# wuxiaolang/Cube_SLAM_wu

Measured on AMD Instinct MI355X. Metric: frames/sec detect_cuboid, higher is better.
Workload: dtype f64

## Files before the change

### cube_slam_wu_amd/csrc/cs_geom.h

```cpp
#pragma once
#include "cs_atan2.h"

namespace cs {

struct V2 {
  double x, y;
};

CS_HD V2 v2(double x, double y) { return V2{x, y}; }
CS_HD double v2_dist(V2 a, V2 b) {
  double dx = a.x - b.x, dy = a.y - b.y;
  return __builtin_sqrt(dx * dx + dy * dy);
}
CS_HD double v2_dist2(V2 a, V2 b) {
  double dx = a.x - b.x, dy = a.y - b.y;
  return dx * dx + dy * dy;
}
static inline double cs_next_up(double x) { long long b = cs_bits(x); return cs_from_bits(b + 1); }
static inline double cs_next_down(double x) { long long b = cs_bits(x); return cs_from_bits(b - 1); }
static inline double sqrt_lt_bound(double t) {
  if (!(t > 0)) return 0.0;
  if (t == __builtin_huge_val()) return t;
  double c = t * t;
  if (c == __builtin_huge_val()) c = 1.7976931348623157e308;
  while (c > 0 && __builtin_sqrt(c) >= t) c = cs_next_down(c);
  while (__builtin_sqrt(c) < t) { if (c >= 1.7976931348623157e308) return __builtin_huge_val(); c = cs_next_up(c); }
  return c;
}
static inline double sqrt_le_bound(double t) {
  if (t != t) return __builtin_huge_val();
  if (t < 0) return -1.0;
  if (t == __builtin_huge_val()) return t;
  const double lt = sqrt_lt_bound(cs_next_up(t));
  if (lt == __builtin_huge_val()) return 1.7976931348623157e308;
  return lt > 0 ? cs_next_down(lt) : 0.0;
}
CS_HD double dmin(double a, double b) { return (b < a) ? b : a; }
CS_HD double dmax(double a, double b) { return (a < b) ? b : a; }
CS_HD double dabs(double a) { return __builtin_fabs(a); }

#define CS_PI 3.14159265358979323846

CS_HD double normalize_to_pi(double a) {
  if (a > CS_PI / 2) return a - CS_PI;
  else if (a < -CS_PI / 2) return a + CS_PI;
  return a;
}

CS_HD bool inside_box(V2 p, double l, double t, double r, double b) { return l <= p.x && p.x <= r && t <= p.y && p.y <= b; }

CS_HD V2 ray_hit_vertical(V2 s, V2 e, double bx, double by0, double by1) {
  V2 hit = v2(-1, -1);
  double dx = e.x - s.x, dy = e.y - s.y;
  if (by0 == by1) {
    double lambd = (by0 - s.y) / dy;
    if (lambd >= 0) {
      V2 t = v2(s.x + lambd * dx, s.y + lambd * dy);
      if ((bx <= t.x) && (t.x <= bx)) { hit = t; hit.y = by0; }
    }
  }
  double lambd = (bx - s.x) / dx;
  if (lambd >= 0) {
    V2 t = v2(s.x + lambd * dx, s.y + lambd * dy);
    if ((by0 <= t.y) && (t.y <= by1)) { hit = t; hit.x = bx; }
  }
  return hit;
}

CS_HD V2 ray_hit_horizontal(V2 s, V2 e, double by, double bx0, double bx1) {
  V2 hit = v2(-1, -1);
  double dx = e.x - s.x, dy = e.y - s.y;
  double lambd = (by - s.y) / dy;
  if (lambd >= 0) {
    V2 t = v2(s.x + lambd * dx, s.y + lambd * dy);
    if ((bx0 <= t.x) && (t.x <= bx1)) { hit = t; hit.y = by; }
  }
  if (bx0 == bx1) {
    double l2 = (bx0 - s.x) / dx;
    if (l2 >= 0) {
      V2 t = v2(s.x + l2 * dx, s.y + l2 * dy);
      if ((by <= t.y) && (t.y <= by)) { hit = t; hit.x = bx0; }
    }
  }
  return hit;
}

CS_HD V2 line_intersect(V2 a1, V2 a2, V2 b1, V2 b2) {
  double X2_X1 = a2.x - a1.x, Y2_Y1 = a2.y - a1.y;
  double X4_X3 = b2.x - b1.x, Y4_Y3 = b2.y - b1.y;
  double X1_X3 = a1.x - b1.x, Y1_Y3 = a1.y - b1.y;
  double u_a = (X4_X3 * Y1_Y3 - Y4_Y3 * X1_X3) / (Y4_Y3 * X2_X1 - X4_X3 * Y2_Y1);
  return v2((a1.x + X2_X1 * u_a) * 1.0, (a1.y + Y2_Y1 * u_a) * 1.0);
}

struct BoxGeom {
  int left, top, right, down;
  int el, et, er, eb;
};

CS_HD int build_corners(const BoxGeom& g, V2 vp1, V2 vp2, V2 vp3, double top_x, int config_id, double short_sq_bound, V2 c[8]) {
  V2 c1 = v2(top_x, (double)g.top);
  int vp1_pos = 0;
  V2 c2 = ray_hit_vertical(vp1, c1, (double)g.right, (double)g.top, (double)g.down);
  if (c2.x == -1) {
    c2 = ray_hit_vertical(vp1, c1, (double)g.left, (double)g.top, (double)g.down);
    if (c2.x != -1) vp1_pos = 2;
  } else {
    vp1_pos = 1;
  }
  if (!(vp1_pos > 0)) return 0;
  if (v2_dist2(c1, c2) < short_sq_bound) return 0;
  V2 c3, c4;
  if (config_id == 1) {
    if (vp1_pos == 1) c4 = ray_hit_vertical(vp2, c1, (double)g.left, (double)g.top, (double)g.down);
    else c4 = ray_hit_vertical(vp2, c1, (double)g.right, (double)g.top, (double)g.down);
    if (c4.y == -1) return 0;
    if (v2_dist2(c1, c4) < short_sq_bound) return 0;
    c3 = line_intersect(vp2, c2, vp1, c4);
    if (!inside_box(c3, g.left, g.top, g.right, g.down)) return 0;
    if ((v2_dist2(c3, c4) < short_sq_bound) || (v2_dist2(c3, c2) < short_sq_bound)) return 0;
  } else {
    if (vp1_pos == 1) c3 = ray_hit_vertical(vp2, c2, (double)g.left, (double)g.top, (double)g.down);
    else c3 = ray_hit_vertical(vp2, c2, (double)g.right, (double)g.top, (double)g.down);
    if (c3.y == -1) return 0;
    if (v2_dist2(c2, c3) < short_sq_bound) return 0;
    c4 = line_intersect(vp1, c3, vp2, c1);
    if (!inside_box(c4, g.left, g.et, g.right, g.eb)) return 0;
    if ((v2_dist2(c3, c4) < short_sq_bound) || (v2_dist2(c4, c1) < short_sq_bound)) return 0;
  }
  V2 c5 = ray_hit_horizontal(vp3, c3, (double)g.down, (double)g.left, (double)g.right);
  if (c5.y == -1) return 0;
  if (v2_dist2(c3, c5) < short_sq_bound) return 0;
  V2 c6 = line_intersect(vp2, c5, vp3, c2);
  if (!inside_box(c6, g.el, g.et, g.er, g.eb)) return 0;
  if ((v2_dist2(c6, c2) < short_sq_bound) || (v2_dist2(c6, c5) < short_sq_bound)) return 0;
  V2 c7 = line_intersect(vp1, c6, vp3, c1);
  if (!inside_box(c7, g.el, g.et, g.er, g.eb)) return 0;
  if ((v2_dist2(c7, c1) < short_sq_bound) || (v2_dist2(c7, c6) < short_sq_bound)) return 0;
  V2 c8 = line_intersect(vp1, c5, vp2, c7);
  if (!inside_box(c8, g.el, g.et, g.er, g.eb)) return 0;
  if ((v2_dist2(c8, c4) < short_sq_bound) || (v2_dist2(c8, c5) < short_sq_bound) || (v2_dist2(c8, c7) < short_sq_bound)) return 0;
  c[0] = c1; c[1] = c2; c[2] = c3; c[3] = c4; c[4] = c5; c[5] = c6; c[6] = c7; c[7] = c8;
  return vp1_pos;
}

CS_HD void rebuild_accepted_corners(const BoxGeom& g, V2 vp1, V2 vp2, V2 vp3, double top_x, int config_id, int vp1_pos, V2 c[8]) {
  const V2 c1 = v2(top_x, (double)g.top);
  const bool right_first = vp1_pos == 1;
  const double side1 = (double)(right_first ? g.right : g.left), side2 = (double)(right_first ? g.left : g.right);
  const bool k1 = config_id == 1;
  V2 c2;
  { const double dx = c1.x - vp1.x, dy = c1.y - vp1.y, lambd = (side1 - vp1.x) / dx; c2 = v2(side1, vp1.y + lambd * dy); }
  const V2 P = k1 ? c1 : c2;
  V2 H;
  { const double dx = P.x - vp2.x, dy = P.y - vp2.y, lambd = (side2 - vp2.x) / dx; H = v2(side2, vp2.y + lambd * dy); }
  const V2 L = line_intersect(k1 ? vp2 : vp1, k1 ? c2 : H, k1 ? vp1 : vp2, k1 ? H : c1);
  const V2 c3 = k1 ? L : H, c4 = k1 ? H : L;
  V2 c5;
  { const double dx = c3.x - vp3.x, dy = c3.y - vp3.y, lambd = ((double)g.down - vp3.y) / dy; c5 = v2(vp3.x + lambd * dx, (double)g.down); }
  const V2 c6 = line_intersect(vp2, c5, vp3, c2);
  const V2 c7 = line_intersect(vp1, c6, vp3, c1);
  const V2 c8 = line_intersect(vp1, c5, vp2, c7);
  c[0] = c1; c[1] = c2; c[2] = c3; c[3] = c4; c[4] = c5; c[5] = c6; c[6] = c7; c[7] = c8;
}

struct RpPose {
  double KinvR[9];
  double R[9];
  double t[3];
  double plane[4];
  double roll, pitch;
};

CS_HD void plane_hit_world(const double* R, const double* t, const double* invK, const double plane[4], double px, double py, double out[3]) {
  double ray[3];
  for (int i = 0; i < 3; i++) ray[i] = (invK[3 * i + 0] * px + invK[3 * i + 1] * py) + invK[3 * i + 2] * 1.0;
  double den = (plane[0] * ray[0] + plane[1] * ray[1]) + plane[2] * ray[2];
  double frac = -plane[3] / den;
  double p[3] = {frac * ray[0], frac * ray[1], frac * ray[2]};
  double w = ((0.0 * p[0] + 0.0 * p[1]) + 0.0 * p[2]) + 1.0 * 1.0;
  for (int i = 0; i < 3; i++) {
    double v = ((R[3 * i + 0] * p[0] + R[3 * i + 1] * p[1]) + R[3 * i + 2] * p[2]) + t[i] * 1.0;
    out[i] = (w != w) ? w : v;
  }
}

CS_HD void lift_to_3d(const V2 c[8], const double* R, const double* t, const double* invK, const double ground_plane[4], double pos[3], double scale[3]) {
  double g[4][3];
  for (int k = 0; k < 4; k++) plane_hit_world(R, t, invK, ground_plane, c[4 + k].x, c[4 + k].y, g[k]);
  double d03[3] = {g[0][0] - g[3][0], g[0][1] - g[3][1], g[0][2] - g[3][2]};
  double d01[3] = {g[0][0] - g[1][0], g[0][1] - g[1][1], g[0][2] - g[1][2]};
  double length_half = __builtin_sqrt((d03[0] * d03[0] + d03[1] * d03[1]) + d03[2] * d03[2]) / 2;
  double width_half = __builtin_sqrt((d01[0] * d01[0] + d01[1] * d01[1]) + d01[2] * d01[2]) / 2;
  double n[3] = {d01[1] * 1.0 - d01[2] * 0.0, d01[2] * 0.0 - d01[0] * 1.0, d01[0] * 0.0 - d01[1] * 0.0};
  double nn = __builtin_sqrt((n[0] * n[0] + n[1] * n[1]) + n[2] * n[2]);
  for (int i = 0; i < 3; i++) n[i] /= nn;
  double dist = -((n[0] * g[0][0] + n[1] * g[0][1]) + n[2] * g[0][2]);
  double pw[4] = {n[0], n[1], n[2], dist};
  if (dist < 0) for (int i = 0; i < 4; i++) pw[i] = -pw[i];
  double ps[4];
  for (int i = 0; i < 3; i++) ps[i] = ((R[0 + i] * pw[0] + R[3 + i] * pw[1]) + R[6 + i] * pw[2]) + 0.0 * pw[3];
  ps[3] = ((t[0] * pw[0] + t[1] * pw[1]) + t[2] * pw[2]) + 1.0 * pw[3];
  double top[3];
  plane_hit_world(R, t, invK, ps, c[1].x, c[1].y, top);
  double height_half = top[2] / 2;
  pos[0] = (((g[0][0] + g[1][0]) + g[2][0]) + g[3][0]) / 4.0;
  pos[1] = (((g[0][1] + g[1][1]) + g[2][1]) + g[3][1]) / 4.0;
  pos[2] = height_half;
  scale[0] = length_half; scale[1] = width_half; scale[2] = height_half;
}

}
```

### cube_slam_wu_amd/csrc/detect_kernels.hip

```cpp
#include <hip/hip_runtime.h>
#include "cs_hip_util.h"

#include <cstdio>
#include <cstdlib>
#include <cstring>

#include "../../include/cubeslam_hip.h"
#include "detect_types.h"

namespace cs {

__device__ __forceinline__ int wave_uniform_i32(int x) { return __builtin_amdgcn_readfirstlane(x); }
__device__ __forceinline__ long long wave_uniform_i64(long long x) {
  const unsigned lo = (unsigned)__builtin_amdgcn_readfirstlane((int)(unsigned)(x & 0xffffffffll)), hi = (unsigned)__builtin_amdgcn_readfirstlane((int)(x >> 32));
  return (long long)(((unsigned long long)hi << 32) | lo);
}
template <typename T>
__device__ __forceinline__ int find_job_wave(const T* __restrict__ prefix, int n, T elem) {
  const T first = sizeof(T) == 8 ? (T)wave_uniform_i64((long long)elem) : (T)wave_uniform_i32((int)elem);
  int lo = 0, hi = n;
  while (hi - lo > 1) {
    const int mid = (lo + hi) >> 1;
    if (prefix[mid] <= first) lo = mid; else hi = mid;
  }
// ... 123 lines not shown
        ch->dir[lane] = make_float2(cosf((float)a), sinf((float)a));
      }
      __builtin_amdgcn_fence(__ATOMIC_ACQ_REL, "wavefront");
      __builtin_amdgcn_wave_barrier();
      unsigned long long mask[K];
#pragma unroll
      for (int k = 0; k < K; k++) mask[k] = 0;
#pragma unroll 4
      for (int u = 0; u < n; u++) {
        const double2 P = ch->xy[u];
        const float2 ud = ch->dir[u];
#pragma unroll
        for (int k = 0; k < K; k++) {
          const float fx = (float)(P.x - vpx[k]), fy = (float)(P.y - vpy[k]);
          const float cr = fabsf(__builtin_fmaf(fx, ud.y, -(fy * ud.x))), dt = fabsf(__builtin_fmaf(fx, ud.x, fy * ud.y));
          const bool out_for_sure = cr > __builtin_fmaf(tan_f[k], dt, 2.0e-6f * (fabsf(fx) + fabsf(fy)));
          mask[k] |= (unsigned long long)(out_for_sure ? 0 : 1) << u;
        }
      }
#pragma unroll
      for (int k = 0; k < K; k++) {
        unsigned long long mk = lane_on ? mask[k] : 0ull;
        while (__any(mk != 0)) {
          if (mk != 0) {
            const int u = __ffsll((long long)mk) - 1;
            mk &= mk - 1;
            const double2 P = ch->xy[u];
            vp_step(mx, my, c0 + u, P.x, P.y, ch->ang[u], vpx[k], vpy[k], thre[k], thre_f[k], R[k]);
          }
        }
      }
    }
  } else {
    const int mm = lane_on ? m : 0;
    for (int i = 0; i < mm; i++) {
      const double X = mx[i], Y = my[i], A = la[i];
#pragma unroll
      for (int k = 0; k < K; k++) vp_step(mx, my, i, X, Y, A, vpx[k], vpy[k], thre[k], thre_f[k], R[k]);
    }
  }
  const double NaN = __builtin_nan("");
#pragma unroll
  for (int k = 0; k < K; k++) {
    const double ang_hi = R[k].have ? la[R[k].i_hi] : NaN, ang_lo = R[k].have ? la[R[k].i_lo] : NaN;
    out[2 * k] = swapped[k] ? ang_lo : ang_hi;
    out[2 * k + 1] = swapped[k] ? ang_hi : ang_lo;
  }
}

enum { VP3_RPCAP = 32 };

template <int MODE, bool UNIFORM>
__device__ __forceinline__ void vp_support_body(const DetectDeviceView& v, const SweepParams& sp, const JobDesc& jd, int j, long long e, bool on, VpChunk* ch) {
  int rp = 0, y = 0;
  if (on) {
    int local = (int)e - jd.vp_off;
    on = local < jd.RP * jd.Y;
    rp = local / jd.Y; y = local - rp * jd.Y;
  }
  double vpx[3] = {0, 0, 0}, vpy[3] = {0, 0, 0};
  if (on) {
    const RpPose* pose = v.rp + jd.rp_off + rp;
    double cy = v.yaw_cos[jd.yaw_off + y], sy = v.yaw_sin[jd.yaw_off + y];
    const double* A = pose->KinvR;
    double d[3][3] = {{cy, sy, 0.0}, {-sy, cy, 0.0}, {0.0, 0.0, 1.0}};
#pragma unroll
    for (int k = 0; k < 3; k++) {
      double h0 = (A[0] * d[k][0] + A[1] * d[k][1]) + A[2] * d[k][2];
      double h1 = (A[3] * d[k][0] + A[4] * d[k][1]) + A[5] * d[k][2];
      double h2 = (A[6] * d[k][0] + A[7] * d[k][1]) + A[8] * d[k][2];
      vpx[k] = h0 / h2;
      vpy[k] = h1 / h2;
    }
    if (MODE == 0) {
      double* vout = v.vp + 6 * e;
      vout[0] = vpx[0]; vout[1] = vpy[0]; vout[2] = vpx[1]; vout[3] = vpy[1]; vout[4] = vpx[2]; vout[5] = vpy[2];
    }
  }
  const double* mx = v.mid_x + jd.line_off;
  const double* my = v.mid_y + jd.line_off;
  const double* la = v.line_angle + jd.line_off;
  double b6[6];
  const double thre[3] = {sp.vp12_thre_rad, sp.vp12_thre_rad, sp.vp3_thre_rad};
  const bool swapped[3] = {false, true, true};
  vp_support_multi<(MODE == 0 ? 3 : 2), UNIFORM>(mx, my, la, jd.m, ch, vpx, vpy, thre, swapped, on, b6);
  if (!on) return;
  if (MODE == 1) { const double* t3 = v.bound3 + 2 * ((size_t)j * VP3_RPCAP + rp); b6[4] = t3[0]; b6[5] = t3[1]; }
  double* bout = v.bound + 6 * e;
#pragma unroll
  for (int q = 0; q < 6; q++) bout[q] = b6[q];
}

template <int MODE>
__global__ __launch_bounds__(256) void vp_support_kernel(DetectDeviceView v, SweepParams sp, int vp_total) {
  long long e = xcd_virtual_block() * blockDim.x + threadIdx.x;
  const bool on = e < vp_total;
  const int j = find_job_wave<int>(v.vp_prefix, v.n_jobs, on ? (int)e : vp_total - 1);
  const int ju = wave_uniform_i32(j);
  __shared__ VpChunk chunk[4];
  if (__all(j == ju)) vp_support_body<MODE, true>(v, sp, v.jobs[ju], ju, e, on, &chunk[threadIdx.x >> 6]);
  else vp_support_body<MODE, false>(v, sp, v.jobs[j], j, e, on, nullptr);
}

__global__ __launch_bounds__(64) void vp3_support_kernel(DetectDeviceView v, SweepParams sp, int rp_stride) {
  const long long e = (long long)blockIdx.x * 64 + threadIdx.x;
  const int j = (int)(e / rp_stride), rp = (int)(e % rp_stride);
  bool on = j < v.n_jobs;
  JobDesc jd{};
  if (on) { jd = v.jobs[j]; on = rp < jd.RP && jd.Y > 0; }
  double vx = 0, vy = 0;
  if (on) {
    const double* A = (v.rp + jd.rp_off + rp)->KinvR;
    double h0 = (A[0] * 0.0 + A[1] * 0.0) + A[2] * 1.0;
    double h1 = (A[3] * 0.0 + A[4] * 0.0) + A[5] * 1.0;
    double h2 = (A[6] * 0.0 + A[7] * 0.0) + A[8] * 1.0;
    vx = h0 / h2; vy = h1 / h2;
  }
  double o2[2];
  const bool swapped3 = true;
  vp_support_multi<1, false>(v.mid_x + jd.line_off, v.mid_y + jd.line_off, v.line_angle + jd.line_off, on ? jd.m : 0, nullptr, &vx, &vy, &sp.vp3_thre_rad, &swapped3, on, o2);
  if (on) { double* t3 = v.bound3 + 2 * ((size_t)j * VP3_RPCAP + rp); t3[0] = o2[0]; t3[1] = o2[1]; }
}

__global__ __launch_bounds__(256) void vp_points_kernel(DetectDeviceView v, int vp_total) {
  long long e = (long long)blockIdx.x * blockDim.x + threadIdx.x;
  int j = find_job_wave<int>(v.vp_prefix, v.n_jobs, e < vp_total ? (int)e : vp_total - 1);
  if (e >= vp_total) return;
  const JobDesc jd = v.jobs[j];
  int local = (int)e - jd.vp_off;
  if (local >= jd.RP * jd.Y) return;
  int rp = local / jd.Y, y = local - rp * jd.Y;
  const RpPose* pose = v.rp + jd.rp_off + rp;
  double cy = v.yaw_cos[jd.yaw_off + y], sy = v.yaw_sin[jd.yaw_off + y];
  const double* A = pose->KinvR;
  double d[3][3] = {{cy, sy, 0.0}, {-sy, cy, 0.0}, {0.0, 0.0, 1.0}};
  double* vout = v.vp + 6 * e;
#pragma unroll
  for (int k = 0; k < 3; k++) {
    double h0 = (A[0] * d[k][0] + A[1] * d[k][1]) + A[2] * d[k][2];
    double h1 = (A[3] * d[k][0] + A[4] * d[k][1]) + A[5] * d[k][2];
    double h2 = (A[6] * d[k][0] + A[7] * d[k][1]) + A[8] * d[k][2];
    vout[2 * k] = h0 / h2;
    vout[2 * k + 1] = h1 / h2;
  }
}

__device__ __forceinline__ int candidate_one(const DetectDeviceView& v, const SweepParams& sp, const JobDesc& jd, long long tid) {
  const unsigned k = (unsigned)(tid - jd.slot_off);
  const unsigned half = (unsigned)jd.RP * (unsigned)jd.Y * (unsigned)jd.T;
  if (k >= 2 * half) { v.flag[tid] = 0; return 0; }
  const int cfg = (k >= half) ? 2 : 1;
  const unsigned rest = (k >= half) ? k - half : k;
  const unsigned ryu = rest / (unsigned)jd.T;
  const int t = (int)(rest - ryu * (unsigned)jd.T);
  const long long slot = jd.slot_off + (long long)rest * 2 + (cfg - 1);
  const bool enabled = (cfg == 1) ? (sp.consider_config_1 != 0) : (sp.consider_config_2 != 0);
  int flag = 0;
  if (enabled) {
    const double* vp = v.vp + 6 * (long long)(jd.vp_off + (int)ryu);
    V2 c[8];
    flag = build_corners(jd.g, v2(vp[0], vp[1]), v2(vp[2], vp[3]), v2(vp[4], vp[5]), (double)v.top_x[jd.top_off + t], cfg, sp.short_sq_bound, c);
  }
  v.flag[slot] = flag;
  return flag;
}

__global__ __launch_bounds__(256) void candidate_kernel(DetectDeviceView v, SweepParams sp, long long slot_total) {
  long long tid = xcd_virtual_block() * blockDim.x + threadIdx.x;
  bool active = tid < slot_total;
  int flag = 0;
  int j = find_job_wave<long long>(v.slot_prefix, v.n_jobs, active ? tid : slot_total - 1);
  const int ju = wave_uniform_i32(j);
  if (__all(j == ju)) {
    if (active) flag = candidate_one(v, sp, v.jobs[ju], tid);
  } else {
    if (active) flag = candidate_one(v, sp, v.jobs[j], tid);
  }
  unsigned long long valid = __ballot(flag != 0);
  if (valid) {
    int lane = threadIdx.x & 63;
    int j0 = __shfl(j, __ffsll((long long)valid) - 1);
    unsigned long long same = __ballot(flag != 0 && j == j0);
    if (same == valid) {
      if (lane == __ffsll((long long)valid) - 1) atomicAdd(&v.job_valid[j0], __popcll(valid));
    } else if (flag != 0) {
      atomicAdd(&v.job_valid[j], 1);
    }
  }
}

enum { COMPACT_PER = 16 };
enum { CC_TRIP = 4096 };
__global__ __launch_bounds__(256) void candidate_compact_kernel(DetectDeviceView v, SweepParams sp) {
  const int j = blockIdx.x;
  if (j >= v.n_jobs) return;
  __shared__ unsigned char s_flag[CC_TRIP];
  __shared__ int wsum[4];
  const JobDesc& jd = v.jobs[j];
  const int tid = threadIdx.x, lane = tid & 63, wid = tid >> 6;
  const int n_vp = jd.RP * jd.Y;
  for (int e = tid; e < n_vp; e += 256) {
    const int rp = e / jd.Y, y = e - rp * jd.Y;
    const RpPose* pose = v.rp + jd.rp_off + rp;
    const double cy = v.yaw_cos[jd.yaw_off + y], sy = v.yaw_sin[jd.yaw_off + y];
    const double* A = pose->KinvR;
    const double d[3][3] = {{cy, sy, 0.0}, {-sy, cy, 0.0}, {0.0, 0.0, 1.0}};
    double* vout = v.vp + 6 * (long long)(jd.vp_off + e);
#pragma unroll
    for (int k = 0; k < 3; k++) {
      const double h0 = (A[0] * d[k][0] + A[1] * d[k][1]) + A[2] * d[k][2];
      const double h1 = (A[3] * d[k][0] + A[4] * d[k][1]) + A[5] * d[k][2];
      const double h2 = (A[6] * d[k][0] + A[7] * d[k][1]) + A[8] * d[k][2];
      vout[2 * k] = h0 / h2;
      vout[2 * k + 1] = h1 / h2;
    }
  }
  __syncthreads();
  const unsigned half = (unsigned)n_vp * (unsigned)jd.T;
  const unsigned Tu = (unsigned)jd.T;
  const bool fast_div = Tu > 1 && (unsigned long long)half * Tu < (1ull << 32);
  const unsigned inv_T = fast_div ? 0xffffffffu / Tu + 1u : 0u;
  const long long base = v.slot_prefix[j];
  long long run = base;
  const unsigned long long below = (1ull << lane) - 1ull;
  const bool en1 = sp.consider_config_1 != 0, en2 = sp.consider_config_2 != 0;
  for (unsigned r0 = 0; r0 < half; r0 += CC_TRIP / 2) {
#pragma unroll 1
    for (int q = 0; q < 16; q++) {
      const int cfg = 1 + (q >> 3);
      const unsigned rl = (unsigned)(q & 7) * 256u + (unsigned)tid, rest = r0 + rl;
      int flag = 0;
      if (rest < half && (cfg == 1 ? en1 : en2)) {
        const unsigned ryu = fast_div ? __umulhi(rest, inv_T) : rest / Tu;
        const int t = (int)(rest - ryu * Tu);
        const double* vp = v.vp + 6 * (long long)(jd.vp_off + (int)ryu);
        V2 c[8];
        flag = build_corners(jd.g, v2(vp[0], vp[1]), v2(vp[2], vp[3]), v2(vp[4], vp[5]), (double)v.top_x[jd.top_off + t], cfg, sp.short_sq_bound, c);
      }
      s_flag[2 * rl + (unsigned)(cfg - 1)] = (unsigned char)flag;
    }
    __syncthreads();
    int f[COMPACT_PER];
    int wcount = 0;
#pragma unroll
    for (int q = 0; q < COMPACT_PER; q++) {
      f[q] = s_flag[wid * (64 * COMPACT_PER) + q * 64 + lane];
      wcount += __popcll(__ballot(f[q] != 0));
    }
    if (lane == 0) wsum[wid] = wcount;
    __syncthreads();
    int woff = 0, total = 0;
#pragma unroll
    for (int w = 0; w < 4; w++) { const int x = wsum[w]; if (w < wid) woff += x; total += x; }
    long long pos0 = run + woff;
    const long long sl0 = base + 2ll * r0 + wid * (64 * COMPACT_PER) + lane;
#pragma unroll
    for (int q = 0; q < COMPACT_PER; q++) {
      const unsigned long long bal = __ballot(f[q] != 0);
      if (f[q] != 0) {
        const long long pos = pos0 + __popcll(bal & below);
        v.c_slot[pos] = sl0 + q * 64;
        v.c_flag[pos] = f[q] | (j << CAND_JOB_SHIFT);
      }
      pos0 += __popcll(bal);
    }
    run += total;
    __syncthreads();
  }
  const int n_valid = (int)(run - base);
  if (tid == 0) { v.job_valid[j] = n_valid; v.job_cbase[j] = base; }
  const int nblk = (n_valid + 255) >> 8;
  if (nblk > 0) {
    __shared__ int s_at;
    if (tid == 0) s_at = atomicAdd(&v.blk_info[0], nblk);
    __syncthreads();
    const int at = s_at, b0 = (int)(base >> 8);
    for (int k = tid; k < nblk; k += 256) {
      const int left = n_valid - 256 * k;
      v.blk_info[2 + 2 * (long long)(at + k)] = b0 + k;
      v.blk_info[3 + 2 * (long long)(at + k)] = left > 256 ? 256 : left;
    }
  }
}

__device__ __forceinline__ int slot_corners(const DetectDeviceView& v, const JobDesc& jd, long long slot, double short_sq_bound, V2 c[8]) {
  const unsigned local = (unsigned)(slot - jd.slot_off);
  const unsigned rest = local >> 1, ryu = rest / (unsigned)jd.T;
  const int t = (int)(rest - ryu * (unsigned)jd.T);
  const double* vp = v.vp + 6 * (long long)(jd.vp_off + (int)ryu);
  return build_corners(jd.g, v2(vp[0], vp[1]), v2(vp[2], vp[3]), v2(vp[4], vp[5]), (double)v.top_x[jd.top_off + t], (int)(local & 1) + 1, short_sq_bound, c);
}
__device__ __forceinline__ void slot_corners16(const DetectDeviceView& v, long long slot, double short_sq_bound, double out16[16]) {
  int lo = 0, hi = v.n_jobs;
  while (hi - lo > 1) { const int mid = (lo + hi) >> 1; if (v.slot_prefix[mid] <= slot) lo = mid; else hi = mid; }
  V2 c[8];
#pragma unroll
  for (int q = 0; q < 8; q++) c[q] = v2(0.0, 0.0);
  slot_corners(v, v.jobs[lo], slot, short_sq_bound, c);
#pragma unroll
  for (int q = 0; q < 8; q++) { out16[q] = c[q].x; out16[8 + q] = c[q].y; }
}

__device__ __forceinline__ int sel(int cfg, int a, int b) { return cfg ? b : a; }

enum { SCORE_JOBS = 4, SCORE_SUB = 128, SCORE_BINS = SCORE_JOBS * SCORE_SUB };
__device__ __forceinline__ unsigned score_udiv(unsigned n, unsigned d, unsigned inv) { return inv ? __umulhi(n, inv) : n / d; }
template <bool CAP>
__global__ __launch_bounds__(256) void score_kernel(DetectDeviceView v, long long slot_total, double short_sq_bound) {
  __shared__ double C16[16][260];
  double (*CXt)[260] = C16, (*CYt)[260] = C16 + 8;
  const bool cap = CAP;
  long long n_valid = cap ? 256ll * v.blk_info[0] : v.job_cbase[v.n_jobs];
  const long long per_xcd = ((n_valid + 255) / 256 + 7) / 8;
  const long long kx = blockIdx.x >> 3;
  if (kx >= per_xcd) return;
  long long base = ((long long)(blockIdx.x & 7) * per_xcd + kx) * blockDim.x;
  if (base >= n_valid) return;
  if (cap) {
    const int* entry = v.blk_info + 2 + 2 * (base >> 8);
    base = 256ll * entry[0];
    n_valid = base + entry[1];
  }
  __shared__ int hist[SCORE_BINS + 1];
  __shared__ int s_src[256], s_job[256], s_flag[256];
  __shared__ long long s_slot[256];
  {
    const int t0 = threadIdx.x;
    for (int b = t0; b <= SCORE_BINS; b += 256) hist[b] = 0;
    __syncthreads();
    const long long i0 = base + t0;
    long long slot0 = 0;
    int j0 = 0;
    int flag0 = 0;
    if (i0 < n_valid) { slot0 = v.c_slot[i0]; flag0 = v.c_flag[i0]; j0 = flag0 >> CAND_JOB_SHIFT; }
    s_slot[t0] = slot0; s_job[t0] = j0; s_flag[t0] = flag0 & CAND_VP_MASK;
    __syncthreads();
    int key = SCORE_BINS;
    if (i0 < n_valid) {
      const int jq = CAP ? __builtin_amdgcn_readfirstlane(s_job[0]) : j0;
      const int T0 = v.jobs[jq].T;
      const unsigned loc = (unsigned)(slot0 - v.jobs[jq].slot_off);
      const int jrel = j0 - s_job[0];
      const unsigned hq = loc >> 1;
      const unsigned qT = CAP ? score_udiv(hq, (unsigned)T0, ((unsigned long long)v.jobs[jq].RP * v.jobs[jq].Y * T0 * T0 < (1ull << 32) && T0 > 1) ? 0xffffffffu / (unsigned)T0 + 1u : 0u) : hq / (unsigned)T0;
      const int sub = (int)(loc & 1) * T0 + (int)(hq - qT * (unsigned)T0);
      key = (jrel < SCORE_JOBS && sub < SCORE_SUB) ? jrel * SCORE_SUB + sub : SCORE_BINS - 1;
    }
    const int rank = atomicAdd(&hist[key], 1);
    __syncthreads();
    if (t0 < 64) {
      constexpr int PER = (SCORE_BINS + 1 + 63) / 64;
      int loc_sum = 0, vals[PER];
#pragma unroll
      for (int q = 0; q < PER; q++) { const int b = t0 * PER + q; vals[q] = b <= SCORE_BINS ? hist[b] : 0; loc_sum += vals[q]; }
      int incl = loc_sum;
#pragma unroll
      for (int o = 1; o < 64; o <<= 1) { const int y = __shfl_up(incl, o); if (t0 >= o) incl += y; }
      int run = incl - loc_sum;
#pragma unroll
      for (int q = 0; q < PER; q++) { const int b = t0 * PER + q; if (b <= SCORE_BINS) hist[b] = run; run += vals[q]; }
    }
    __syncthreads();
    s_src[hist[key] + rank] = t0;
    __syncthreads();
  }
  const int mine = s_src[threadIdx.x];
  const JobDesc& jd = v.jobs[CAP ? __builtin_amdgcn_readfirstlane(s_job[0]) : s_job[mine]];
  const long long i = base + mine;
  if (i >= n_valid) return;
  const long long slot = s_slot[mine];
  const unsigned local = (unsigned)(slot - jd.slot_off);
  const int cfg = (int)(local & 1);
  const unsigned inv_T = (CAP && jd.T > 1 && (unsigned long long)jd.RP * jd.Y * jd.T * jd.T < (1ull << 32)) ? 0xffffffffu / (unsigned)jd.T + 1u : 0u;
  const unsigned inv_Y = (CAP && jd.Y > 1 && (unsigned long long)jd.RP * jd.Y * jd.Y < (1ull << 32)) ? 0xffffffffu / (unsigned)jd.Y + 1u : 0u;
  const int ry = (int)score_udiv(local >> 1, (unsigned)jd.T, inv_T);
  const int rp = (int)score_udiv((unsigned)ry, (unsigned)jd.Y, inv_Y);
  const int tx = threadIdx.x;
  const double ox = (double)jd.g.el, oy = (double)jd.g.et;
  const float* __restrict__ map = v.maps + jd.map_off;
  {
    V2 cb[8];
    const unsigned rest = local >> 1;
    const double* vp = v.vp + 6 * (long long)(jd.vp_off + ry);
    rebuild_accepted_corners(jd.g, v2(vp[0], vp[1]), v2(vp[2], vp[3]), v2(vp[4], vp[5]), (double)v.top_x[jd.top_off + (int)(rest - (unsigned)ry * (unsigned)jd.T)], cfg + 1,
                             s_flag[mine], cb);
#pragma unroll
    for (int q = 0; q < 8; q++) { CXt[q][tx] = cb[q].x; CYt[q][tx] = cb[q].y; }
  }
  double bnd[6];
  {
    const double* bound = v.bound + 6 * (long long)(jd.vp_off + ry);
#pragma unroll
    for (int q = 0; q < 6; q++) bnd[q] = bound[q];
  }
  float sum_dist = 0;
  const unsigned long long EA = cfg ? 0x004213210ull : 0x443213210ull, EB = cfg ? 0x005450321ull : 0x577450321ull;
  const unsigned long long EW = cfg ? 0x004332222ull : 0x222222222ull;
  const int n_edges = cfg ? 7 : 9;
  const int map_w = jd.map_w;
  constexpr int EU = 3;
  const bool wave_has_cfg1 = __any(cfg == 0);
#pragma unroll 1
  for (int e0 = 0; e0 < n_edges; e0 += EU) {
    float dv[EU][11];
#pragma unroll
    for (int u = 0; u < EU; u++) {
      const int e = e0 + u;
      if (u > 0 && e0 == 6 && !wave_has_cfg1) {
#pragma unroll
        for (int s = 0; s < 11; s++) dv[u][s] = 0.0f;
        continue;
      }
      const int a = (int)((EA >> (4 * e)) & 7), b = (int)((EB >> (4 * e)) & 7);
      const double x1 = CXt[a][tx] - ox, y1 = CYt[a][tx] - oy, x2 = CXt[b][tx] - ox, y2 = CYt[b][tx] - oy;
#pragma unroll
      for (int s = 0; s < 11; s++) {
        double sx, sy;
        if (s == 0) { sx = x2; sy = y2; }
        else if (s == 10) { sx = x1; sy = y1; }
        else if (s == 5) { sx = (x1 + x2) * 0.5; sy = (y1 + y2) * 0.5; }
        else { const double w = (double)s / 10.0; sx = w * x1 + (1 - w) * x2; sy = w * y1 + (1 - w) * y2; }
        dv[u][s] = map[(unsigned)(__mul24((int)sy, map_w) + (int)sx)];
      }
    }
#pragma unroll
    for (int u = 0; u < EU; u++) {
      const int e = e0 + u;
      const float wt = 0.5f * (float)(int)((EW >> (4 * e)) & 7);
      const bool on = e < n_edges;
#pragma unroll
      for (int s = 0; s < 11; s++) { const float nx = sum_dist + dv[u][s] * wt; sum_dist = on ? nx : sum_dist; }
    }
  }
  double total = 0;
  const double not_found_penalty = 30.0 / 180.0 * CS_PI * 2;
  const int ID1[3][4] = {{0, 1, 7, 4}, {3, 0, 4, 5}, {3, 7, 1, 5}}, ID2[3][4] = {{0, 1, 2, 3}, {3, 0, 4, 5}, {2, 4, 1, 5}};
#pragma unroll
  for (int k = 0; k < 3; k++) {
    double b0 = bnd[2 * k], b1 = bnd[2 * k + 1];
    bool v0 = !(b0 != b0), v1 = !(b1 != b1);
    if (v0 || v1) {
#pragma unroll
      for (int ee = 0; ee < 2; ee++) {
        int pa = sel(cfg, ID1[k][2 * ee], ID2[k][2 * ee]), pb = sel(cfg, ID1[k][2 * ee + 1], ID2[k][2 * ee + 1]);
        double ang = normalize_to_pi(cs_atan2(CYt[pb][tx] - CYt[pa][tx], CXt[pb][tx] - CXt[pa][tx]));
        double best = 100;
        if (v0) { double t = dabs(ang - b0); t = dmin(t, CS_PI - t); if (t < best) best = t; }
        if (v1) { double t = dabs(ang - b1); t = dmin(t, CS_PI - t); if (t < best) best = t; }
        total = total + best;
      }
    } else {
      total = total + not_found_penalty;
    }
  }
  V2 c[8];
#pragma unroll
  for (int q = 0; q < 8; q++) c[q] = v2(CXt[q][tx], CYt[q][tx]);
  const RpPose* pose = v.rp + jd.rp_off + rp;
  double p3[3], s3[3];
  lift_to_3d(c, pose->R, pose->t, v.invK + 9 * jd.frame, pose->plane, p3, s3);
  int flag = s_flag[mine];
  if (s3[0] < 0 || s3[1] < 0 || s3[2] < 0) flag |= CAND_NEG_SCALE;
  v.c_flag[i] = flag;
  v.c_dist[i] = (double)sum_dist / jd.diag;
  v.c_angle[i] = total;
  v.c_skew[i] = dmax(s3[0], s3[1]) / dmin(s3[0], s3[1]);
}

__global__ __launch_bounds__(1024) void scan_jobs_kernel(const int* job_valid, long long* job_cbase, int n_jobs) {
  __shared__ long long wsum[16];
  __shared__ long long carry_s;
  if (threadIdx.x == 0) carry_s = 0;
  __syncthreads();
  int lane = threadIdx.x & 63, wid = threadIdx.x >> 6;
  for (int base = 0; base < n_jobs; base += 1024) {
    int i = base + threadIdx.x;
    long long x = (i < n_jobs) ? job_valid[i] : 0;
    long long incl = x;
#pragma unroll
    for (int o = 1; o < 64; o <<= 1) {
      long long y = __shfl_up(incl, o);
      if (lane >= o) incl += y;
    }
    if (lane == 63) wsum[wid] = incl;
    __syncthreads();
    long long woff = 0;
    for (int w = 0; w < wid; w++) woff += wsum[w];
    long long carry = carry_s;
    if (i < n_jobs) job_cbase[i] = carry + woff + incl - x;
    __syncthreads();
    if (threadIdx.x == 1023) carry_s = carry + woff + incl;
    __syncthreads();
  }
  if (threadIdx.x == 0) job_cbase[n_jobs] = carry_s;
}

__global__ __launch_bounds__(256) void compact_kernel(DetectDeviceView v) {
  int j = blockIdx.x;
  if (j >= v.n_jobs) return;
  __shared__ int wsum[4];
  const long long s0 = v.slot_prefix[j], s1 = v.slot_prefix[j + 1];
  long long run = v.job_cbase[j];
  const int lane = threadIdx.x & 63, wid = threadIdx.x >> 6;
  const unsigned long long below = (1ull << lane) - 1ull;
  for (long long base = s0; base < s1; base += 256 * COMPACT_PER) {
    const long long w0 = base + (long long)wid * (64 * COMPACT_PER) + lane;
    int f[COMPACT_PER];
    int wcount = 0;
#pragma unroll
    for (int q = 0; q < COMPACT_PER; q++) {
      const long long sl = w0 + q * 64;
      f[q] = (sl < s1) ? v.flag[sl] : 0;
      wcount += __popcll(__ballot(f[q] != 0));
    }
    if (lane == 0) wsum[wid] = wcount;
    __syncthreads();
    int woff = 0, total = 0;
#pragma unroll
    for (int w = 0; w < 4; w++) { const int x = wsum[w]; if (w < wid) woff += x; total += x; }
    long long pos0 = run + woff;
#pragma unroll
    for (int q = 0; q < COMPACT_PER; q++) {
      const unsigned long long bal = __ballot(f[q] != 0);
      if (f[q] != 0) {
        const long long pos = pos0 + __popcll(bal & below);
        v.c_slot[pos] = w0 + q * 64;
        v.c_flag[pos] = f[q] | (j << CAND_JOB_SHIFT);
      }
      pos0 += __popcll(bal);
    }
    run += total;
    __syncthreads();
  }
}

__global__ __launch_bounds__(256) void compact_count_kernel(DetectDeviceView v, int* __restrict__ cnt, int maxc) {
  const int j = blockIdx.x, c = blockIdx.y;
  __shared__ int wsum[4];
  const long long end = v.slot_prefix[j + 1], s0 = v.slot_prefix[j] + (long long)c * (256 * COMPACT_PER), s1 = (s0 + 256 * COMPACT_PER < end) ? s0 + 256 * COMPACT_PER : end;
  int n = 0;
  for (long long sl = s0 + threadIdx.x; sl < s1; sl += 256) n += v.flag[sl] != 0;
#pragma unroll
  for (int o = 32; o > 0; o >>= 1) n += __shfl_down(n, o);
  if ((threadIdx.x & 63) == 0) wsum[threadIdx.x >> 6] = n;
  __syncthreads();
  if (threadIdx.x == 0) cnt[(size_t)j * maxc + c] = wsum[0] + wsum[1] + wsum[2] + wsum[3];
}
__global__ __launch_bounds__(256) void compact_chunk_kernel(DetectDeviceView v, const int* __restrict__ cnt, int maxc) {
  const int j = blockIdx.x, c = blockIdx.y;
  __shared__ int wsum[4];
  const long long s1 = v.slot_prefix[j + 1], base = v.slot_prefix[j] + (long long)c * (256 * COMPACT_PER);
  if (base >= s1) return;
  long long run = v.job_cbase[j];
  for (int q = 0; q < c; q++) run += cnt[(size_t)j * maxc + q];
  const int lane = threadIdx.x & 63, wid = threadIdx.x >> 6;
  const unsigned long long below = (1ull << lane) - 1ull;
  const long long w0 = base + (long long)wid * (64 * COMPACT_PER) + lane;
  int f[COMPACT_PER];
  int wcount = 0;
#pragma unroll
  for (int q = 0; q < COMPACT_PER; q++) {
    const long long sl = w0 + q * 64;
    f[q] = (sl < s1) ? v.flag[sl] : 0;
    wcount += __popcll(__ballot(f[q] != 0));
  }
  if (lane == 0) wsum[wid] = wcount;
  __syncthreads();
  int woff = 0;
#pragma unroll
  for (int w = 0; w < 4; w++) if (w < wid) woff += wsum[w];
  long long pos0 = run + woff;
#pragma unroll
  for (int q = 0; q < COMPACT_PER; q++) {
    const unsigned long long bal = __ballot(f[q] != 0);
    if (f[q] != 0) {
      const long long pos = pos0 + __popcll(bal & below);
      v.c_slot[pos] = w0 + q * 64;
      v.c_flag[pos] = f[q] | (j << CAND_JOB_SHIFT);
    }
    pos0 += __popcll(bal);
  }
}

__global__ __launch_bounds__(64) void gather_corners_kernel(DetectDeviceView v, double short_sq_bound, const long long* slots, int n, double* out) {
  int w = blockIdx.x * blockDim.x + threadIdx.x;
  if (w >= n) return;
  long long s = slots[w];
  double c16[16];
#pragma unroll
  for (int q = 0; q < 16; q++) c16[q] = 0.0;
  if (s >= 0) slot_corners16(v, s, short_sq_bound, c16);
#pragma unroll
  for (int q = 0; q < 16; q++) out[16 * (size_t)w + q] = c16[q];
}


__device__ __forceinline__ unsigned long long order_key(double x) {
  unsigned long long b = (unsigned long long)__double_as_longlong(x);
  return (b >> 63) ? ~b : (b | 0x8000000000000000ull);
}

template <int NT>
__device__ void block_radix_select2(const double* __restrict__ a, const double* __restrict__ b, int n, int r, unsigned* hist , unsigned long long* bcast ,
                                    unsigned long long* key_a, unsigned long long* key_b) {
  unsigned long long prefix[2] = {0, 0}, mask = 0;
  int rr2[2] = {r, r};
  for (int pass = 0; pass < 8; pass++) {
    const int shift = 56 - 8 * pass;
    for (int q = threadIdx.x; q < 512; q += NT) hist[q] = 0;
    __syncthreads();
    for (int i = threadIdx.x; i < n; i += NT) {
      const unsigned long long ka = order_key(a[i]), kb = order_key(b[i]);
      if ((ka & mask) == prefix[0]) atomicAdd(&hist[(unsigned)(ka >> shift) & 255u], 1u);
      if ((kb & mask) == prefix[1]) atomicAdd(&hist[256 + ((unsigned)(kb >> shift) & 255u)], 1u);
    }
    __syncthreads();
    for (int col = 0; col < 2; col++) {
      if ((int)(threadIdx.x >> 6) != (NT >= 128 ? col : 0)) continue;
      const int lane = threadIdx.x & 63;
      const unsigned* h = hist + 256 * col;
      unsigned c0 = h[4 * lane], c1 = h[4 * lane + 1], c2 = h[4 * lane + 2], c3 = h[4 * lane + 3];
      unsigned tot = c0 + c1 + c2 + c3, incl = tot;
#pragma unroll
      for (int o = 1; o < 64; o <<= 1) { unsigned y = __shfl_up(incl, o); if (lane >= o) incl += y; }
      unsigned excl = incl - tot;
      const unsigned rk = (unsigned)rr2[col];
      if (rk >= excl && rk < incl) {
        unsigned rr = rk - excl, d;
        if (rr < c0) { d = 0; }
        else if (rr < c0 + c1) { d = 1; rr -= c0; }
        else if (rr < c0 + c1 + c2) { d = 2; rr -= c0 + c1; }
        else { d = 3; rr -= c0 + c1 + c2; }
        bcast[2 * col] = (unsigned long long)(4 * lane + d);
        bcast[2 * col + 1] = rr;
      }
    }
    __syncthreads();
    prefix[0] |= bcast[0] << shift; prefix[1] |= bcast[2] << shift;
    mask |= 255ull << shift;
    rr2[0] = (int)bcast[1]; rr2[1] = (int)bcast[3];
    __syncthreads();
  }
  *key_a = prefix[0]; *key_b = prefix[1];
}

template <int NT>
__device__ __forceinline__ double block_reduce_min(double v, double* sh) {
#pragma unroll
  for (int o = 32; o > 0; o >>= 1) { double y = __shfl_down(v, o); v = (y < v) ? y : v; }
  if ((threadIdx.x & 63) == 0) sh[threadIdx.x >> 6] = v;
  __syncthreads();
  double r = sh[0];
  for (int w = 1; w < NT / 64; w++) r = (sh[w] < r) ? sh[w] : r;
  __syncthreads();
  return r;
}
template <int NT>
__device__ __forceinline__ double block_reduce_max(double v, double* sh) {
#pragma unroll
  for (int o = 32; o > 0; o >>= 1) { double y = __shfl_down(v, o); v = (y > v) ? y : v; }
  if ((threadIdx.x & 63) == 0) sh[threadIdx.x >> 6] = v;
  __syncthreads();
  double r = sh[0];
  for (int w = 1; w < NT / 64; w++) r = (sh[w] > r) ? sh[w] : r;
  __syncthreads();
  return r;
}
template <int NT>
__device__ __forceinline__ int block_reduce_sum_i(int v, int* sh) {
#pragma unroll
  for (int o = 32; o > 0; o >>= 1) v += __shfl_down(v, o);
  if ((threadIdx.x & 63) == 0) sh[threadIdx.x >> 6] = v;
  __syncthreads();
  int r = sh[0];
  for (int w = 1; w < NT / 64; w++) r += sh[w];
  __syncthreads();
  return r;
}

struct JobCut {
  double vd, va;
  double dmin, dmax, amin, amax;
  int use_angle, n_keep, V;
  int tie;
};

enum { RW_K = 28, RW_CAP = 64 * RW_K, RW_BATCH = 8 };
__device__ __forceinline__ bool rank_box_fits_wave(const DetectDeviceView& v, int j0, int nj) {
  bool fits = true;
  for (int h = 0; h < nj; h++) fits = fits && v.job_valid[j0 + h] <= (int)RW_CAP;
  return fits;
}
__device__ __forceinline__ double rank_combined_score(const JobCut& c, const RankParams& rp, double d, double a, double sk, double* score_out) {
  double score;
  if (c.n_keep > 1) {
    double dn = (d - c.dmin) / (c.dmax - c.dmin);
    double an = ((c.amax - c.amin) > 0) ? (a - c.amin) / (c.amax - c.amin) : a;
    score = (dn + rp.w_angle * an) / (1 + rp.w_angle);
  } else {
    score = (d + rp.w_angle * a) / (1 + rp.w_angle);
  }
  double skew_error = rp.w_skew * dmax(sk - rp.nominal_skew, 0.0);
  if (sk > rp.max_cut_skew) skew_error = 100;
  *score_out = score;
  return score + rp.w_skew * skew_error;
}
enum { RANK_STAGE = 1536, RANK_THREADS_DEFAULT = 256 };
enum { RANK_STAGE_BIG = 9216, RANK_THREADS_BIG = 1024 };
template <int NT, bool DYN>
__device__ __forceinline__ void rank_block_body(const DetectDeviceView& v, const RankView& rv, const RankParams& rp, int stage_cap, int box) {
  __shared__ unsigned hist[512];
  __shared__ unsigned long long bcast[4];
  __shared__ double shd[NT / 64 > 4 ? NT / 64 : 4];
  __shared__ int shi[NT / 64 > 4 ? NT / 64 : 4];
  __shared__ JobCut cuts[3];
  __shared__ int s_fallback;
  __shared__ double sD_fixed[DYN ? 1 : RANK_STAGE], sA_fixed[DYN ? 1 : RANK_STAGE];
  extern __shared__ double rank_dyn_lds[];
  double* const sD = DYN ? rank_dyn_lds : sD_fixed;
  double* const sA = DYN ? rank_dyn_lds + stage_cap : sA_fixed;
  const int STAGE = DYN ? stage_cap : (int)RANK_STAGE;
  const int j0 = rv.box_job0[box], nj = rv.box_njobs[box];
  if (threadIdx.x == 0) s_fallback = 0;
  __syncthreads();
  const double INF = __builtin_huge_val();
  for (int h = 0; h < nj; h++) {
    int j = j0 + h;
    long long c0 = v.job_cbase[j];
    int V = v.job_valid[j];
    const double* D = v.c_dist + c0;
    const double* A = v.c_angle + c0;
    if (V <= STAGE) {
      __syncthreads();
      for (int i = threadIdx.x; i < V; i += NT) { sD[i] = D[i]; sA[i] = A[i]; }
      __syncthreads();
      D = sD; A = sA;
    }
    double vd = INF, va = INF;
    int use_angle = 0, tie = 0, bn_keep = 0;
    if (V > 4) {
      int bn = (int)round((double)((float)V) / 3.0 * 2.0);
      bn_keep = bn - 1;
      unsigned long long kd, ka;
      block_radix_select2<NT>(D, A, V, bn - 2, hist, bcast, &kd, &ka);
      int cd = 0, ca = 0, nan = 0;
      for (int i = threadIdx.x; i < V; i += NT) {
        double d = D[i], a = A[i];
        cd += order_key(d) <= kd; ca += order_key(a) <= ka;
        nan += (d != d) || (a != a);
      }
      cd = block_reduce_sum_i<NT>(cd, shi); ca = block_reduce_sum_i<NT>(ca, shi); nan = block_reduce_sum_i<NT>(nan, shi);
      if (nan && threadIdx.x == 0) s_fallback = 1;
      tie = (cd != bn - 1);
      use_angle = (ca == bn - 1);
      double md = -INF, ma = -INF;
      for (int i = threadIdx.x; i < V; i += NT) {
        if (order_key(D[i]) <= kd) md = (D[i] > md) ? D[i] : md;
        if (order_key(A[i]) <= ka) ma = (A[i] > ma) ? A[i] : ma;
      }
      vd = block_reduce_max<NT>(md, shd);
      va = block_reduce_max<NT>(ma, shd);
    }
    double dmin = 1e6, dmax = -1, amin = 1e6, amax = -1;
    int nk = 0;
    for (int i = threadIdx.x; i < V; i += NT) {
      double d = D[i], a = A[i];
      bool keep = (d <= vd) && (!use_angle || a <= va);
      if (keep) {
        nk++;
// ... 1073 lines not shown
```

Before: 545,000.

## Specialize score kernel per wave-uniform config and dedupe corner endpoint samples

Scoring is split into a templated score_proposal, picked by whether all lanes in a wave share the same box configuration. The uniform paths fully unroll the edge lists at compile time and sample each cube corner's map pixel only once, reused by every edge touching it, instead of re-reading endpoints per edge. Mixed waves keep the generic loop. The negative-scale check is also narrowed to the third scale component, which changes semantics unless the other two are known non-negative.

New measurement: 533,200. 2.2% lower.

```diff
diff --git a/cube_slam_wu_amd/csrc/cs_geom.h b/cube_slam_wu_amd/csrc/cs_geom.h
--- a/cube_slam_wu_amd/csrc/cs_geom.h
+++ b/cube_slam_wu_amd/csrc/cs_geom.h
@@ -144,11 +144,12 @@
   return vp1_pos;
 }
 
+template <int CONFIG = 0>
 CS_HD void rebuild_accepted_corners(const BoxGeom& g, V2 vp1, V2 vp2, V2 vp3, double top_x, int config_id, int vp1_pos, V2 c[8]) {
   const V2 c1 = v2(top_x, (double)g.top);
   const bool right_first = vp1_pos == 1;
   const double side1 = (double)(right_first ? g.right : g.left), side2 = (double)(right_first ? g.left : g.right);
-  const bool k1 = config_id == 1;
+  const bool k1 = CONFIG ? CONFIG == 1 : config_id == 1;
   V2 c2;
   { const double dx = c1.x - vp1.x, dy = c1.y - vp1.y, lambd = (side1 - vp1.x) / dx; c2 = v2(side1, vp1.y + lambd * dy); }
   const V2 P = k1 ? c1 : c2;
diff --git a/cube_slam_wu_amd/csrc/detect_kernels.hip b/cube_slam_wu_amd/csrc/detect_kernels.hip
--- a/cube_slam_wu_amd/csrc/detect_kernels.hip
+++ b/cube_slam_wu_amd/csrc/detect_kernels.hip
@@ -449,6 +449,147 @@
 }
 
 __device__ __forceinline__ int sel(int cfg, int a, int b) { return cfg ? b : a; }
+__host__ __device__ constexpr unsigned long long score_edges_a(int cfg) { return cfg ? 0x004213210ull : 0x443213210ull; }
+__host__ __device__ constexpr unsigned long long score_edges_b(int cfg) { return cfg ? 0x005450321ull : 0x577450321ull; }
+__host__ __device__ constexpr unsigned long long score_edges_w(int cfg) { return cfg ? 0x004332222ull : 0x222222222ull; }
+__host__ __device__ constexpr int score_n_edges(int cfg) { return cfg ? 7 : 9; }
+__host__ __device__ constexpr int score_nibble(unsigned long long tab, int e) { return (int)((tab >> (4 * e)) & 7); }
+__host__ __device__ constexpr unsigned score_corner_mask(int cfg, int e_begin, int e_end) {
+  unsigned m = 0;
+  for (int e = e_begin; e < e_end && e < score_n_edges(cfg); e++) m |= (1u << score_nibble(score_edges_a(cfg), e)) | (1u << score_nibble(score_edges_b(cfg), e));
+  return m;
+}
+constexpr int SCORE_EU = 3;
+
+__device__ __forceinline__ float score_sample(const float* __restrict__ map, int map_w, int s, double x1, double y1, double x2, double y2) {
+  double sx, sy;
+  if (s == 0) { sx = x2; sy = y2; }
+  else if (s == 10) { sx = x1; sy = y1; }
+  else if (s == 5) { sx = (x1 + x2) * 0.5; sy = (y1 + y2) * 0.5; }
+  else { const double w = (double)s / 10.0; sx = w * x1 + (1 - w) * x2; sy = w * y1 + (1 - w) * y2; }
+  return map[(unsigned)(__mul24((int)sy, map_w) + (int)sx)];
+}
+
+template <int CFG, int E0>
+__device__ __forceinline__ void score_trip(const float* __restrict__ map, int map_w, double ox, double oy, const double (*CXt)[260], const double (*CYt)[260], int tx,
+                                           float (&pix)[8], float& sum_dist) {
+  constexpr int NE = score_n_edges(CFG);
+  constexpr unsigned fresh = score_corner_mask(CFG, E0, E0 + SCORE_EU) & ~score_corner_mask(CFG, 0, E0);
+#pragma unroll
+  for (int q = 0; q < 8; q++)
+    if ((fresh >> q) & 1) { const double x = CXt[q][tx] - ox, y = CYt[q][tx] - oy; pix[q] = score_sample(map, map_w, 0, x, y, x, y); }
+  float dv[SCORE_EU][9];
+#pragma unroll
+  for (int u = 0; u < SCORE_EU; u++) {
+    if (E0 + u >= NE) continue;
+    const int a = score_nibble(score_edges_a(CFG), E0 + u), b = score_nibble(score_edges_b(CFG), E0 + u);
+    const double x1 = CXt[a][tx] - ox, y1 = CYt[a][tx] - oy, x2 = CXt[b][tx] - ox, y2 = CYt[b][tx] - oy;
+#pragma unroll
+    for (int s = 1; s < 10; s++) dv[u][s - 1] = score_sample(map, map_w, s, x1, y1, x2, y2);
+  }
+#pragma unroll
+  for (int u = 0; u < SCORE_EU; u++) {
+    if (E0 + u >= NE) continue;
+    const int a = score_nibble(score_edges_a(CFG), E0 + u), b = score_nibble(score_edges_b(CFG), E0 + u), w2 = score_nibble(score_edges_w(CFG), E0 + u);
+    const float wt = 0.5f * (float)w2;
+#pragma unroll
+    for (int s = 0; s < 11; s++) {
+      const float d = s == 0 ? pix[b] : s == 10 ? pix[a] : dv[u][s - 1];
+      if (w2 == 2) sum_dist = sum_dist + d;
+      else sum_dist = sum_dist + d * wt;
+    }
+  }
+  __builtin_amdgcn_sched_barrier(0);
+}
+
+template <int CFG>
+__device__ __forceinline__ void score_proposal(const DetectDeviceView& v, const JobDesc& jd, long long i, unsigned local, int ry, int rp, int vp1_pos, double (*CXt)[260], double (*CYt)[260]) {
+  const int cfg = CFG < 0 ? (int)(local & 1) : CFG;
+  const int tx = threadIdx.x;
+  const double ox = (double)jd.g.el, oy = (double)jd.g.et;
+  const float* __restrict__ map = v.maps + jd.map_off;
+  {
+    V2 cb[8];
+    const unsigned rest = local >> 1;
+    const double* vp = v.vp + 6 * (long long)(jd.vp_off + ry);
+    rebuild_accepted_corners<CFG < 0 ? 0 : CFG + 1>(jd.g, v2(vp[0], vp[1]), v2(vp[2], vp[3]), v2(vp[4], vp[5]), (double)v.top_x[jd.top_off + (int)(rest - (unsigned)ry * (unsigned)jd.T)],
+                                                    cfg + 1, vp1_pos, cb);
+#pragma unroll
+    for (int q = 0; q < 8; q++) { CXt[q][tx] = cb[q].x; CYt[q][tx] = cb[q].y; }
+  }
+  double bnd[6];
+  {
+    const double* bound = v.bound + 6 * (long long)(jd.vp_off + ry);
+#pragma unroll
+    for (int q = 0; q < 6; q++) bnd[q] = bound[q];
+  }
+  float sum_dist = 0;
+  const int map_w = jd.map_w;
+  if constexpr (CFG >= 0) {
+    float pix[8];
+    score_trip<CFG, 0>(map, map_w, ox, oy, CXt, CYt, tx, pix, sum_dist);
+    score_trip<CFG, SCORE_EU>(map, map_w, ox, oy, CXt, CYt, tx, pix, sum_dist);
+    score_trip<CFG, 2 * SCORE_EU>(map, map_w, ox, oy, CXt, CYt, tx, pix, sum_dist);
+    static_assert(3 * SCORE_EU >= score_n_edges(0) && 3 * SCORE_EU >= score_n_edges(1), "three trips cover both edge lists");
+  } else {
+    const unsigned long long EA = score_edges_a(cfg), EB = score_edges_b(cfg), EW = score_edges_w(cfg);
+    const int n_edges = score_n_edges(cfg);
+    constexpr int EU = SCORE_EU;
+#pragma unroll 1
+    for (int e0 = 0; e0 < n_edges; e0 += EU) {
+      float dv[EU][11];
+#pragma unroll
+      for (int u = 0; u < EU; u++) {
+        const int e = e0 + u;
+        const int a = score_nibble(EA, e), b = score_nibble(EB, e);
+        const double x1 = CXt[a][tx] - ox, y1 = CYt[a][tx] - oy, x2 = CXt[b][tx] - ox, y2 = CYt[b][tx] - oy;
+#pragma unroll
+        for (int s = 0; s < 11; s++) dv[u][s] = score_sample(map, map_w, s, x1, y1, x2, y2);
+      }
+#pragma unroll
+      for (int u = 0; u < EU; u++) {
+        const int e = e0 + u;
+        const float wt = 0.5f * (float)score_nibble(EW, e);
+        const bool on = e < n_edges;
+#pragma unroll
+        for (int s = 0; s < 11; s++) { const float nx = sum_dist + dv[u][s] * wt; sum_dist = on ? nx : sum_dist; }
+      }
+    }
+  }
+  double total = 0;
+  const double not_found_penalty = 30.0 / 180.0 * CS_PI * 2;
+  const int ID1[3][4] = {{0, 1, 7, 4}, {3, 0, 4, 5}, {3, 7, 1, 5}}, ID2[3][4] = {{0, 1, 2, 3}, {3, 0, 4, 5}, {2, 4, 1, 5}};
+#pragma unroll
+  for (int k = 0; k < 3; k++) {
+    double b0 = bnd[2 * k], b1 = bnd[2 * k + 1];
+    bool v0 = !(b0 != b0), v1 = !(b1 != b1);
+    if (v0 || v1) {
+#pragma unroll
+      for (int ee = 0; ee < 2; ee++) {
+        int pa = sel(cfg, ID1[k][2 * ee], ID2[k][2 * ee]), pb = sel(cfg, ID1[k][2 * ee + 1], ID2[k][2 * ee + 1]);
+        double ang = normalize_to_pi(cs_atan2(CYt[pb][tx] - CYt[pa][tx], CXt[pb][tx] - CXt[pa][tx]));
+        double best = 100;
+        if (v0) { double t = dabs(ang - b0); t = dmin(t, CS_PI - t); if (t < best) best = t; }
+        if (v1) { double t = dabs(ang - b1); t = dmin(t, CS_PI - t); if (t < best) best = t; }
+        total = total + best;
+      }
+    } else {
+      total = total + not_found_penalty;
+    }
+  }
+  V2 c[8];
+#pragma unroll
+  for (int q = 0; q < 8; q++) c[q] = v2(CXt[q][tx], CYt[q][tx]);
+  const RpPose* pose = v.rp + jd.rp_off + rp;
+  double p3[3], s3[3];
+  lift_to_3d(c, pose->R, pose->t, v.invK + 9 * jd.frame, pose->plane, p3, s3);
+  int flag = vp1_pos;
+  if (s3[2] < 0) flag |= CAND_NEG_SCALE;
+  v.c_flag[i] = flag;
+  v.c_dist[i] = (double)sum_dist / jd.diag;
+  v.c_angle[i] = total;
+  v.c_skew[i] = dmax(s3[0], s3[1]) / dmin(s3[0], s3[1]);
+}
 
 enum { SCORE_JOBS = 4, SCORE_SUB = 128, SCORE_BINS = SCORE_JOBS * SCORE_SUB };
 __device__ __forceinline__ unsigned score_udiv(unsigned n, unsigned d, unsigned inv) { return inv ? __umulhi(n, inv) : n / d; }
@@ -522,96 +663,10 @@
   const unsigned inv_Y = (CAP && jd.Y > 1 && (unsigned long long)jd.RP * jd.Y * jd.Y < (1ull << 32)) ? 0xffffffffu / (unsigned)jd.Y + 1u : 0u;
   const int ry = (int)score_udiv(local >> 1, (unsigned)jd.T, inv_T);
   const int rp = (int)score_udiv((unsigned)ry, (unsigned)jd.Y, inv_Y);
-  const int tx = threadIdx.x;
-  const double ox = (double)jd.g.el, oy = (double)jd.g.et;
-  const float* __restrict__ map = v.maps + jd.map_off;
-  {
-    V2 cb[8];
-    const unsigned rest = local >> 1;
-    const double* vp = v.vp + 6 * (long long)(jd.vp_off + ry);
-    rebuild_accepted_corners(jd.g, v2(vp[0], vp[1]), v2(vp[2], vp[3]), v2(vp[4], vp[5]), (double)v.top_x[jd.top_off + (int)(rest - (unsigned)ry * (unsigned)jd.T)], cfg + 1,
-                             s_flag[mine], cb);
-#pragma unroll
-    for (int q = 0; q < 8; q++) { CXt[q][tx] = cb[q].x; CYt[q][tx] = cb[q].y; }
-  }
-  double bnd[6];
-  {
-    const double* bound = v.bound + 6 * (long long)(jd.vp_off + ry);
-#pragma unroll
-    for (int q = 0; q < 6; q++) bnd[q] = bound[q];
-  }
-  float sum_dist = 0;
-  const unsigned long long EA = cfg ? 0x004213210ull : 0x443213210ull, EB = cfg ? 0x005450321ull : 0x577450321ull;
-  const unsigned long long EW = cfg ? 0x004332222ull : 0x222222222ull;
-  const int n_edges = cfg ? 7 : 9;
-  const int map_w = jd.map_w;
-  constexpr int EU = 3;
-  const bool wave_has_cfg1 = __any(cfg == 0);
-#pragma unroll 1
-  for (int e0 = 0; e0 < n_edges; e0 += EU) {
-    float dv[EU][11];
-#pragma unroll
-    for (int u = 0; u < EU; u++) {
-      const int e = e0 + u;
-      if (u > 0 && e0 == 6 && !wave_has_cfg1) {
-#pragma unroll
-        for (int s = 0; s < 11; s++) dv[u][s] = 0.0f;
-        continue;
-      }
-      const int a = (int)((EA >> (4 * e)) & 7), b = (int)((EB >> (4 * e)) & 7);
-      const double x1 = CXt[a][tx] - ox, y1 = CYt[a][tx] - oy, x2 = CXt[b][tx] - ox, y2 = CYt[b][tx] - oy;
-#pragma unroll
-      for (int s = 0; s < 11; s++) {
-        double sx, sy;
-        if (s == 0) { sx = x2; sy = y2; }
-        else if (s == 10) { sx = x1; sy = y1; }
-        else if (s == 5) { sx = (x1 + x2) * 0.5; sy = (y1 + y2) * 0.5; }
-        else { const double w = (double)s / 10.0; sx = w * x1 + (1 - w) * x2; sy = w * y1 + (1 - w) * y2; }
-        dv[u][s] = map[(unsigned)(__mul24((int)sy, map_w) + (int)sx)];
-      }
-    }
-#pragma unroll
-    for (int u = 0; u < EU; u++) {
-      const int e = e0 + u;
-      const float wt = 0.5f * (float)(int)((EW >> (4 * e)) & 7);
-      const bool on = e < n_edges;
-#pragma unroll
-      for (int s = 0; s < 11; s++) { const float nx = sum_dist + dv[u][s] * wt; sum_dist = on ? nx : sum_dist; }
-    }
-  }
-  double total = 0;
-  const double not_found_penalty = 30.0 / 180.0 * CS_PI * 2;
-  const int ID1[3][4] = {{0, 1, 7, 4}, {3, 0, 4, 5}, {3, 7, 1, 5}}, ID2[3][4] = {{0, 1, 2, 3}, {3, 0, 4, 5}, {2, 4, 1, 5}};
-#pragma unroll
-  for (int k = 0; k < 3; k++) {
-    double b0 = bnd[2 * k], b1 = bnd[2 * k + 1];
-    bool v0 = !(b0 != b0), v1 = !(b1 != b1);
-    if (v0 || v1) {
-#pragma unroll
-      for (int ee = 0; ee < 2; ee++) {
-        int pa = sel(cfg, ID1[k][2 * ee], ID2[k][2 * ee]), pb = sel(cfg, ID1[k][2 * ee + 1], ID2[k][2 * ee + 1]);
-        double ang = normalize_to_pi(cs_atan2(CYt[pb][tx] - CYt[pa][tx], CXt[pb][tx] - CXt[pa][tx]));
-        double best = 100;
-        if (v0) { double t = dabs(ang - b0); t = dmin(t, CS_PI - t); if (t < best) best = t; }
-        if (v1) { double t = dabs(ang - b1); t = dmin(t, CS_PI - t); if (t < best) best = t; }
-        total = total + best;
-      }
-    } else {
-      total = total + not_found_penalty;
-    }
-  }
-  V2 c[8];
-#pragma unroll
-  for (int q = 0; q < 8; q++) c[q] = v2(CXt[q][tx], CYt[q][tx]);
-  const RpPose* pose = v.rp + jd.rp_off + rp;
-  double p3[3], s3[3];
-  lift_to_3d(c, pose->R, pose->t, v.invK + 9 * jd.frame, pose->plane, p3, s3);
-  int flag = s_flag[mine];
-  if (s3[0] < 0 || s3[1] < 0 || s3[2] < 0) flag |= CAND_NEG_SCALE;
-  v.c_flag[i] = flag;
-  v.c_dist[i] = (double)sum_dist / jd.diag;
-  v.c_angle[i] = total;
-  v.c_skew[i] = dmax(s3[0], s3[1]) / dmin(s3[0], s3[1]);
+  const bool has_cfg1 = __any(cfg == 0), has_cfg2 = __any(cfg != 0);
+  if (!has_cfg2) score_proposal<0>(v, jd, i, local, ry, rp, s_flag[mine], CXt, CYt);
+  else if (!has_cfg1) score_proposal<1>(v, jd, i, local, ry, rp, s_flag[mine], CXt, CYt);
+  else score_proposal<-1>(v, jd, i, local, ry, rp, s_flag[mine], CXt, CYt);
 }
 
 __global__ __launch_bounds__(1024) void scan_jobs_kernel(const int* job_valid, long long* job_cbase, int n_jobs) {
```
